# anerisheth19/CNN-MobileNet-V1-implementation-on-AWS-FPGA-using-OpenCL

Hardware: AMD Instinct MI355X
Metric: images/sec MobileNet-V1 1.0x224 fp32, batch 256; per-stage HBM GB/s vs roofline (higher is better)
Workload: dtype f32

## Files before the change

cnn-mobilenet-v1-implementation-on-aws-fpga-using-opencl_amd/csrc/mbn_abi.hip:

```cpp
#include "mbn_internal.h"

#include <initializer_list>
#include <new>

mbn_tunables g_mbn_tune;

namespace {

struct Span { const void *p; double bytes; const char *what; };

int span_check(mbn_context *ctx, const Span *sp, int n)
{
    std::lock_guard<std::mutex> lk(ctx->mu);
    if (ctx->allocs.empty()) return MBN_OK;
    for (int i = 0; i < n; i++) {
        if (!sp[i].p || sp[i].bytes <= 0) continue;
        const uintptr_t a = (uintptr_t)sp[i].p;
        auto it = ctx->allocs.upper_bound(a);
        if (it == ctx->allocs.begin()) continue;
        --it;
        if (a >= it->first + it->second) continue;
        const double room = (double)(it->first + it->second - a);
        if (sp[i].bytes > room) {
            snprintf(ctx->last_error, sizeof(ctx->last_error), "%s: call touches %.0f bytes, %.0f left in its %zu-byte mbn_alloc buffer",
// ... 1163 lines not shown
                              const void *fc_bias, int batch, int rows, int cols, int channels, int classes, int k, void *workspace,
                              size_t workspace_bytes, void *stream)
{
    if (!ctx || !topk_idx_i32 || !topk_prob_f32 || !logits || !in || !fc_w || !workspace || batch <= 0 || rows <= 0 || cols <= 0 || channels <= 0 ||
        classes <= 0 || k < 1 || k > 8)
        return MBN_EINVAL;
    if (batch > 4 || channels < 64 || channels > 1024 || (channels % 64) != 0 || classes > 1024) return MBN_EUNSUPPORTED;
    if (workspace_bytes < mbn_pool_fc_ws_bytes(channels, classes)) return MBN_EINVAL;
    hipStream_t s = stream ? (hipStream_t)stream : ctx->stream;
    MBN_SPANS(ctx, { in, 4.0 * batch * rows * cols * channels, "classifier_tail_fused input" }, { logits, 4.0 * batch * classes, "classifier_tail_fused logits" },
              { fc_w, 4.0 * classes * channels, "classifier_tail_fused filter" }, { workspace, (double)mbn_pool_fc_ws_bytes(channels, classes), "classifier_tail_fused workspace" },
              { probs, 4.0 * batch * classes, "classifier_tail_fused probs" }, { topk_idx_i32, 4.0 * batch * k, "classifier_tail_fused idx" },
              { topk_prob_f32, 4.0 * batch * k, "classifier_tail_fused prob" });
    Scope sc(ctx, s);
    return sc.finish(mbn_launch_f32_pool_fc(ctx, s, (float *)logits, (const float *)in, (const float *)fc_w, (const float *)fc_bias, workspace,
                                            batch, rows * cols, channels, classes, k, (float *)probs, (int32_t *)topk_idx_i32, (float *)topk_prob_f32));
}

static int stem_fused_impl(mbn_context *ctx, void *out, const void *image, const void *w1, const void *s1, const void *b1,
                           const void *wd, const void *s2, const void *b2, const void *wp, const void *s3, const void *b3,
                           int batch, int rows, int cols, int c1, int c3, void *stream, int in_u8, int bf16)
{
    if (!ctx || !out || !image) return MBN_EINVAL;
    hipStream_t s = stream ? (hipStream_t)stream : ctx->stream;
    if (mbn_stem_envelope_hw(batch, rows, cols, c1, c3) != MBN_OK) return MBN_EUNSUPPORTED;
    MBN_SPANS(ctx, { image, (in_u8 ? 1.0 : 4.0) * batch * rows * cols * 3, "stem image" },
              { out, (bf16 ? 2.0 : 4.0) * batch * (rows / 2) * (cols / 2) * c3, "stem output" });
    if (check_ptrs({ w1, s1, b1, wd, s2, b2, wp, s3, b3 }) != MBN_OK) return MBN_EUNSUPPORTED;
    if (((uintptr_t)out % 16) != 0 || ((uintptr_t)image % (in_u8 ? 2 : 8)) != 0) return MBN_EINVAL;
    Scope sc(ctx, s);
    return sc.finish(mbn_launch_f32_stem(ctx, s, (float *)out, (const float *)image, (const float *)w1, (const float *)s1,
                                         (const float *)b1, (const float *)wd, (const float *)s2, (const float *)b2,
                                         (const float *)wp, (const float *)s3, (const float *)b3, batch, rows, cols, c1, c3, in_u8, bf16));
}

int mbn_stem_fused_hw(mbn_context *ctx, void *out, const void *image, const void *w1, const void *s1, const void *b1,
                      const void *wd, const void *s2, const void *b2, const void *wp, const void *s3, const void *b3,
                      int batch, int rows, int cols, int c1, int c3, int flags, void *stream)
{
    if (flags & ~(MBN_STEM_IN_U8 | MBN_STEM_BF16)) return MBN_EINVAL;
    return stem_fused_impl(ctx, out, image, w1, s1, b1, wd, s2, b2, wp, s3, b3, batch, rows, cols, c1, c3, stream,
                           (flags & MBN_STEM_IN_U8) != 0, (flags & MBN_STEM_BF16) != 0);
}

int mbn_stem_fused(mbn_context *ctx, void *out, const void *image, const void *w1, const void *s1, const void *b1,
                   const void *wd, const void *s2, const void *b2, const void *wp, const void *s3, const void *b3,
                   int batch, int res, int c1, int c3, void *stream)
{
    return mbn_stem_fused_hw(ctx, out, image, w1, s1, b1, wd, s2, b2, wp, s3, b3, batch, res, res, c1, c3, 0, stream);
}

int mbn_stem_fused_u8(mbn_context *ctx, void *out, const void *image_u8, const void *w1, const void *s1, const void *b1,
                      const void *wd, const void *s2, const void *b2, const void *wp, const void *s3, const void *b3,
                      int batch, int res, int c1, int c3, void *stream)
{
    return mbn_stem_fused_hw(ctx, out, image_u8, w1, s1, b1, wd, s2, b2, wp, s3, b3, batch, res, res, c1, c3, MBN_STEM_IN_U8, stream);
}

int mbn_stem_fused_ex(mbn_context *ctx, void *out, const void *image, const void *w1, const void *s1, const void *b1,
                      const void *wd, const void *s2, const void *b2, const void *wp, const void *s3, const void *b3,
                      int batch, int res, int c1, int c3, int flags, void *stream)
{
    return mbn_stem_fused_hw(ctx, out, image, w1, s1, b1, wd, s2, b2, wp, s3, b3, batch, res, res, c1, c3, flags, stream);
}

int mbn_dwpw_fused(mbn_context *ctx, void *out, const void *in, const void *wd, const void *s2, const void *b2,
                   const void *wp, const void *s3, const void *b3, int batch, int in_rows, int in_cols, int out_rows,
                   int out_cols, int cin, int cout, int stride, int pad_top, int pad_left, void *stream)
{
    if (!ctx) return MBN_EINVAL;
    hipStream_t s = stream ? (hipStream_t)stream : ctx->stream;
    const mbn_block_shape sh = { batch, in_rows, in_cols, out_rows, out_cols, cin, cout, stride, pad_top, pad_left };
    const mbn_block_params p = { wd, s2, b2, wp, s3, b3 };
    int rc = check_ptrs({ in, wd, s2, b2, wp, s3, b3, out });
    if (rc == MBN_OK) rc = mbn_block_envelope(&sh, MBN_DT_F32);
    if (rc != MBN_OK) return rc;
    MBN_SPANS(ctx, { in, 4.0 * batch * in_rows * in_cols * cin, "dwpw input" },
              { out, 4.0 * batch * out_rows * out_cols * cout, "dwpw output" }, { wd, 36.0 * cin, "dwpw depthwise filter" },
              { wp, 4.0 * cin * cout, "dwpw pointwise filter" });
    Scope sc(ctx, s);
    if (g_mbn_tune.pw_emul != 0 && g_mbn_tune.dwpw_variant == 0 && mbn_launch_f32_dwpw2_x6(ctx, s, sh, out, in, p) == MBN_OK)
        return sc.finish(MBN_OK);
    const int dv = g_mbn_tune.dwpw_variant;
    if ((dv == 11 || dv >= 300 || (dv == 0 && MBN_DWPW3_DEFAULT(stride, cin))) && mbn_f32_dwpw3_eligible(ctx, sh))
        return sc.finish(mbn_launch_f32_dwpw3(ctx, s, sh, out, in, p));
    const long tiles256 = (((long)batch * out_rows * out_cols + 127) / 128) * (cout / 256);
    const bool small = tiles256 < ctx->num_cus;
    if (dv != 1 && (dv >= 2 || (cout % 256) != 0 || small || stride == 2))
        return sc.finish(mbn_launch_f32_dwpw2(ctx, s, sh, out, in, p));
    return sc.finish(mbn_launch_f32_dwpw(ctx, s, sh, out, in, p));
}

int mbn_blocks_resident_bf16(mbn_context *ctx, void *out, const void *in, const mbn_block_params *blocks, int nblocks, int batch,
                             int rows, int cols, int channels, void *stream)
{
    if (!ctx || !out || !in || !blocks || batch <= 0) return MBN_EINVAL;
    const mbn_block_shape sh = { batch, rows, cols, rows, cols, channels, channels, 1, 1, 1 };
    if (mbn_resident_envelope(&sh, nblocks) != MBN_OK) return MBN_EUNSUPPORTED;
    hipStream_t s = stream ? (hipStream_t)stream : ctx->stream;
    const double act = 2.0 * batch * rows * cols * channels;
    MBN_SPANS(ctx, { in, act, "resident blocks input" }, { out, act, "resident blocks output" });
    for (int i = 0; i < nblocks; i++) {
        if (!blocks[i].wd || !blocks[i].s2 || !blocks[i].b2 || !blocks[i].wp_bf16 || !blocks[i].s3 || !blocks[i].b3) return MBN_EINVAL;
        MBN_SPANS(ctx, { blocks[i].wd, 36.0 * channels, "resident blocks depthwise filter" }, { blocks[i].wp_bf16, 2.0 * channels * channels, "resident blocks pointwise filter" },
                  { blocks[i].s2, 4.0 * channels, "resident blocks scale" }, { blocks[i].b3, 4.0 * channels, "resident blocks shift" });
    }
    int rc = check_ptrs({ out, in });
    for (int i = 0; i < nblocks && rc == MBN_OK; i++) rc = check_ptrs(blocks[i]);
    if (rc != MBN_OK) return rc;
    Scope sc(ctx, s);
    return sc.finish(mbn_launch_bf16_res_blocks(ctx, s, out, in, blocks, nblocks, batch, rows, cols));
}

int mbn_tail_resident_bf16(mbn_context *ctx, void *out, const void *in, const mbn_block_params *blocks, int batch, int rows, int cols, int c0, int c1,
                           void *stream)
{
    if (!ctx || !out || !in || !blocks || batch <= 0) return MBN_EINVAL;
    const mbn_block_shape b0 = { batch, rows, cols, rows / 2, cols / 2, c0, c1, 2, 0, 0 };
    const mbn_block_shape b1 = { batch, rows / 2, cols / 2, rows / 2, cols / 2, c1, c1, 1, 1, 1 };
    if (mbn_tail_envelope(&b0, &b1) != MBN_OK) return MBN_EUNSUPPORTED;
    hipStream_t s = stream ? (hipStream_t)stream : ctx->stream;
    MBN_SPANS(ctx, { in, 2.0 * batch * rows * cols * c0, "resident tail input" }, { out, 2.0 * batch * c1, "resident tail output" });
    for (int i = 0; i < 2; i++) {
        if (!blocks[i].wd || !blocks[i].s2 || !blocks[i].b2 || !blocks[i].wp_bf16 || !blocks[i].s3 || !blocks[i].b3) return MBN_EINVAL;
        const int ci = i ? c1 : c0;
        MBN_SPANS(ctx, { blocks[i].wd, 36.0 * ci, "resident tail depthwise filter" }, { blocks[i].wp_bf16, 2.0 * ci * c1, "resident tail pointwise filter" },
                  { blocks[i].s2, 4.0 * ci, "resident tail scale" }, { blocks[i].b2, 4.0 * ci, "resident tail shift" },
                  { blocks[i].s3, 4.0 * c1, "resident tail scale" }, { blocks[i].b3, 4.0 * c1, "resident tail shift" });
    }
    int rc = ((uintptr_t)out % 2) ? MBN_EUNSUPPORTED : check_ptrs({ in });
    for (int i = 0; i < 2 && rc == MBN_OK; i++) rc = check_ptrs(blocks[i]);
    if (rc != MBN_OK) return rc;
    Scope sc(ctx, s);
    return sc.finish(mbn_launch_bf16_tail(ctx, s, out, in, blocks, batch, rows, cols));
}

int mbn_dwpw_fused_bf16(mbn_context *ctx, void *out, const void *in, const void *wd, const void *s2, const void *b2,
                        const void *wp_bf16, const void *s3, const void *b3, int batch, int in_rows, int in_cols, int out_rows,
                        int out_cols, int cin, int cout, int stride, int pad_top, int pad_left, void *stream)
{
    if (!ctx) return MBN_EINVAL;
    hipStream_t s = stream ? (hipStream_t)stream : ctx->stream;
    const mbn_block_shape sh = { batch, in_rows, in_cols, out_rows, out_cols, cin, cout, stride, pad_top, pad_left };
    const mbn_block_params p = { wd, s2, b2, wp_bf16, s3, b3 };
    int rc = check_ptrs({ in, wd, s2, b2, wp_bf16, s3, b3, out });
    if (rc == MBN_OK) rc = mbn_block_envelope(&sh, MBN_DT_BF16);
    if (rc != MBN_OK) return rc;
    MBN_SPANS(ctx, { in, 2.0 * batch * in_rows * in_cols * cin, "dwpw input" },
              { out, 2.0 * batch * out_rows * out_cols * cout, "dwpw output" }, { wd, 36.0 * cin, "dwpw depthwise filter" },
              { wp_bf16, 2.0 * cin * cout, "dwpw pointwise filter" });
    Scope sc(ctx, s);
#ifdef MBN_LAB
    if (g_mbn_tune.dwpw_variant == 1 && (cout % 128) == 0 && (cin % 64) == 0)
        return sc.finish(mbn_launch_bf16_dwpw(ctx, s, sh, out, in, p));
#endif
    return sc.finish(mbn_launch_bf16_dwpw2(ctx, s, sh, out, in, p));
}

int mbn_convert_f32_to_bf16(mbn_context *ctx, void *dst_bf16, const void *src_f32, size_t count, void *stream)
{
    if (!ctx || !dst_bf16 || !src_f32) return MBN_EINVAL;
    if (count == 0) return MBN_OK;
    hipStream_t s = stream ? (hipStream_t)stream : ctx->stream;
    MBN_SPANS(ctx, { src_f32, 4.0 * count, "convert source" }, { dst_bf16, 2.0 * count, "convert destination" });
    Scope sc(ctx, s);
    return sc.finish(mbn_launch_convert(ctx, s, dst_bf16, src_f32, count, 1));
}
// ... 46 lines not shown
```

cnn-mobilenet-v1-implementation-on-aws-fpga-using-opencl_amd/csrc/mbn_f32_dwpw3.hip:

```cpp
#include "mbn_internal.h"
#include "mbn_epilogue.h"
#include "mbn_block_window.h"

namespace {

constexpr int BN3 = 128;
constexpr int WT = 32;
constexpr unsigned PO_INVALID = MBN_OFF_BAD_ROW;

struct DwPw3Args {
    float *out;
    const float *in, *wd, *s2, *b2, *wp, *s3, *b3;
    long m;
    int h, w, ho, wo;
    int cout;
    int pad_top, pad_left;
    int nh;
    int tiles;
    unsigned in_bytes;
    int rsh;
    unsigned pb, bi;
    unsigned pb_m, pb_s, bi_m, bi_s;
    float inv_pb, inv_bi;
    int dbg;
};

__device__ __forceinline__ f4 bn_relu6_pk(f4 a, f4 s, f4 b)
{
    const f4 v = __builtin_elementwise_fma(a, s, b);
    return f4{ mbn_relu6(v.x), mbn_relu6(v.y), mbn_relu6(v.z), mbn_relu6(v.w) };
}

template <int S, int CIN, int KS, int ABL, int SCHED = 0, bool B64 = false>
__global__ __launch_bounds__(512) void dwpw3_f32(DwPw3Args a)
{
    constexpr int XC = S + 3;
    constexpr int NS = CIN / 16;
    constexpr int AH = KS / 16;
    constexpr int LPP = KS / 4;
    constexpr int LDB = B64 ? CIN + 2 : CIN + 4;
    constexpr int ABUF = WT * KS;
    static_assert(NS >= 4 && (CIN % 64) == 0 && (KS == 16 || KS == 32), "Cin in multiples of 64");
    __shared__ __attribute__((aligned(16))) float lds[BN3 * LDB + 8 * AH * ABUF + 11 * CIN + 2 * BN3 + 8 * 32];
    float *const wp_s = lds, *const a_s = wp_s + BN3 * LDB, *const wd_s = a_s + 8 * AH * ABUF, *const sb_s = wd_s + 9 * CIN;
    float *const sc3_s = sb_s + 2 * CIN, *const sh3_s = sc3_s + BN3;
    unsigned *const po_s = reinterpret_cast<unsigned *>(sh3_s + BN3);
    const int dbg = ABL < 0 ? a.dbg : ABL;

    const int tid = threadIdx.x, lane = tid & 63;
    const int wave_u = __builtin_amdgcn_readfirstlane(tid >> 6);
    const unsigned ptot = (unsigned)(a.m >> 1);

    const int xcd = (int)blockIdx.x & 7, j = (int)blockIdx.x >> 3, g8 = (int)gridDim.x >> 3;
    const int slice = j % a.nh, jm = j / a.nh, JM = g8 / a.nh;
    const int n0 = slice * BN3;
    const int r0 = (int)(((long)a.tiles * xcd) >> 3), r1 = (int)(((long)a.tiles * (xcd + 1)) >> 3);
    const int per_round = JM * 8;
    const int full = (r1 - r0) / per_round, rem = (r1 - r0) - full * per_round;
    const int slot = jm * 8 + wave_u, eslot = wave_u * JM + jm;
    const int ntile = full + (eslot < rem ? 1 : 0);
    auto tile_at = [&](int i) __attribute__((always_inline)) { return i < full ? r0 + i * per_round + slot : r0 + full * per_round + eslot; };

    {
        constexpr int NP = BN3 * (CIN / 4) / 512;
        f4 pc[NP];
#pragma unroll
        for (int i = 0; i < NP; i++) {
            const int p = tid + i * 512, r = p / (CIN / 4), u = p % (CIN / 4);
            const int ch = n0 + 4 * (r & 31) + (r >> 5);
            pc[i] = *reinterpret_cast<const f4 *>(a.wp + (size_t)ch * CIN + 4 * u);
        }
        f4 tp[3];
        const int ti = tid * 4;
#pragma unroll
        for (int i = 0; i < 3; i++) {
            const int idx = ti + i * 2048;
            tp[i] = idx < 9 * CIN ? *reinterpret_cast<const f4 *>(a.wd + idx) : f4{ 0.f, 0.f, 0.f, 0.f };
        }
        f4 sb[2] = { f4{ 0.f, 0.f, 0.f, 0.f }, f4{ 0.f, 0.f, 0.f, 0.f } };
        if (ti < CIN) {
            sb[0] = *reinterpret_cast<const f4 *>(a.s2 + ti);
            sb[1] = *reinterpret_cast<const f4 *>(a.b2 + ti);
        }
#pragma unroll
        for (int i = 0; i < NP; i++) {
            const int p = tid + i * 512, r = p / (CIN / 4), u = p % (CIN / 4);
            if constexpr (B64) {
                *reinterpret_cast<f2 *>(wp_s + r * LDB + 4 * u) = f2{ pc[i].x, pc[i].y };
                *reinterpret_cast<f2 *>(wp_s + r * LDB + 4 * u + 2) = f2{ pc[i].z, pc[i].w };
            } else *reinterpret_cast<f4 *>(wp_s + r * LDB + 4 * u) = pc[i];
        }
#pragma unroll
        for (int i = 0; i < 3; i++) {
            const int idx = ti + i * 2048;
            if (idx < 9 * CIN) *reinterpret_cast<f4 *>(wd_s + idx) = tp[i];
        }
        if (ti < CIN) {
            *reinterpret_cast<f4 *>(sb_s + ti) = sb[0];
            *reinterpret_cast<f4 *>(sb_s + CIN + ti) = sb[1];
        }
    }
    if (tid < BN3) { sc3_s[tid] = a.s3[n0 + tid]; sh3_s[tid] = a.b3[n0 + tid]; }
    __syncthreads();
    if (ntile == 0) return;

    const int qh = lane / LPP, cl = lane % LPP;
    const int li = lane & 31, lh = lane >> 5;
    const __amdgpu_buffer_rsrc_t irsrc = mbn_make_rsrc(a.in, a.in_bytes);
    const __amdgpu_buffer_rsrc_t orsrc = mbn_make_rsrc(a.out, (unsigned)(a.m * a.cout * 4));
    float *const a_w = a_s + wave_u * (AH * ABUF);
    unsigned *const po_w = po_s + wave_u * 32;
    auto aw_at = [&](const int hh) __attribute__((always_inline)) {
        const int row = 8 * hh * (AH - 1) + qh;
        return KS == 16 ? row * KS + ((cl ^ ((row >> 2) & 3)) << 2) : row * KS + ((cl ^ ((row >> 1) & 7)) << 2);
    };
    const int aw[2] = { aw_at(0), aw_at(1) };
    auto fra_at = [&](const int u) __attribute__((always_inline)) {
        return KS == 16 ? li * KS + (((u + lh) ^ ((li >> 2) & 3)) << 2) : li * KS + (((u + lh) ^ ((li >> 1) & 7)) << 2);
    };
    const int fra[4] = { fra_at(0), fra_at(2), fra_at(KS == 32 ? 4 : 0), fra_at(KS == 32 ? 6 : 2) };
    const float *const bl01 = wp_s + li * LDB + lh * 4;
    const float *const bl23 = bl01 + 64 * LDB;
    const float *const wk = wd_s + cl * 4;

    constexpr bool SEP = S == 2 && AH == 2;
    unsigned off[SEP ? 1 : AH][SEP ? 1 : 3][SEP ? 1 : XC];
    unsigned rowv_k[SEP ? AH : 1][3], colv_k[SEP ? AH : 1][XC];
    auto set_offsets = [&](unsigned p0, const int hh, int pslot) __attribute__((always_inline)) {
        const unsigned bg0 = a.pb_m ? __umulhi(p0, a.pb_m) >> a.pb_s : p0;
        const unsigned i0 = p0 - bg0 * a.pb;
        const unsigned im0 = a.bi_m ? __umulhi(bg0, a.bi_m) >> a.bi_s : bg0;
        const unsigned b0 = bg0 - im0 * a.bi;
        const unsigned qq = (unsigned)(8 * hh * (AH - 1) + qh);
        const unsigned i1 = i0 + qq;
        const unsigned dq = (unsigned)__builtin_fmaf((float)i1, a.inv_pb, 0.5f * a.inv_pb);
        const unsigned i = i1 - (unsigned)__mul24((int)dq, (int)a.pb);
        const unsigned b1 = b0 + dq;
        const unsigned dn = (unsigned)__builtin_fmaf((float)b1, a.inv_bi, 0.5f * a.inv_bi);
        const unsigned band = b1 - (unsigned)__mul24((int)dn, (int)a.bi);
        const unsigned n = im0 + dn;
        const unsigned y = (band << a.rsh) + (i & ((1u << a.rsh) - 1u)), x = (i >> a.rsh) << 1;
        const bool mok = p0 + qq < ptot;
        unsigned rowv[3], colv[XC];
        mbn_window_rowcol<S>(rowv, colv, a, (unsigned)CIN * 4u, (unsigned)(cl * 16), n, y, x, mok);
        if constexpr (SEP) {
#pragma unroll
            for (int dy = 0; dy < 3; dy++) rowv_k[hh][dy] = rowv[dy];
#pragma unroll
            for (int jj = 0; jj < XC; jj++) colv_k[hh][jj] = colv[jj];
        } else {
#pragma unroll
            for (int dy = 0; dy < 3; dy++)
#pragma unroll
                for (int jj = 0; jj < XC; jj++) off[hh][dy][jj] = rowv[dy] + colv[jj];
        }
        const unsigned opix = (unsigned)__mul24((int)(n * (unsigned)a.ho + y), a.wo) + x;
        const unsigned po = mok ? opix * ((unsigned)a.cout * 4u) : PO_INVALID;
        unsigned lid;
        asm volatile("v_mbcnt_lo_u32_b32 %0, -1, 0\n\tv_mbcnt_hi_u32_b32 %0, -1, %0" : "=v"(lid));
        if ((lid % LPP) == 0) po_w[pslot * 16 + 8 * hh * (AH - 1) + (int)(lid / LPP)] = po;
    };
    auto set_offsets_tile = [&](unsigned p0, int pslot) __attribute__((always_inline)) {
#pragma unroll
        for (int hh = 0; hh < AH; hh++) set_offsets(p0, hh, pslot);
    };

    f4 xr[3][XC];
    auto ldx_row = [&](const int u, const int dy) __attribute__((always_inline)) {
        const int hh = AH == 2 ? (u & 1) : 0, cb = AH == 2 ? (u >> 1) * 128 : u * 64;
#pragma unroll
        for (int jj = 0; jj < XC; jj++)
            xr[dy][jj] = __builtin_bit_cast(f4, __builtin_amdgcn_raw_buffer_load_b128(irsrc, (SEP ? rowv_k[hh][dy] + colv_k[hh][jj] : off[SEP ? 0 : hh][SEP ? 0 : dy][SEP ? 0 : jj]) + (unsigned)cb, 0, 0));
    };
    f4 wrow[3], wss[2];
    auto ldw_row = [&](const int u, const int dy) __attribute__((always_inline)) {
        if (dbg & 32) return;
        const int cf = AH == 2 ? (u >> 1) * 32 : u * 16;
#pragma unroll
        for (int dx = 0; dx < 3; dx++) wrow[dx] = *reinterpret_cast<const f4 *>(wk + cf + (dy * 3 + dx) * CIN);
    };
    auto ldw_ss = [&](const int u) __attribute__((always_inline)) {
        if (dbg & 32) return;
        const int cf = AH == 2 ? (u >> 1) * 32 : u * 16;
        wss[0] = *reinterpret_cast<const f4 *>(wk + 9 * CIN + cf);
        wss[1] = *reinterpret_cast<const f4 *>(wk + 10 * CIN + cf);
    };
    f4 dacc0 = f4{ 0.f, 0.f, 0.f, 0.f }, dacc1 = dacc0;
    auto dw_row = [&](const int u, const int dy) __attribute__((always_inline)) {
        if (dy == 0) {
            dacc0 = f4{ 0.f, 0.f, 0.f, 0.f };
            dacc1 = dacc0;
        }
        if (!(dbg & 2)) {
#pragma unroll
            for (int dx = 0; dx < 3; dx++) {
                dacc0 = __builtin_elementwise_fma(xr[dy][dx], wrow[dx], dacc0);
                dacc1 = __builtin_elementwise_fma(xr[dy][dx + S], wrow[dx], dacc1);
            }
        }
        if (dy < 2) ldw_row(u, dy + 1);
        else ldw_ss(u);
    };
    auto dw_fin = [&](const int u) __attribute__((always_inline)) {
        if (dbg & 64) return;
        const int hh = AH == 2 ? (u & 1) : 0, buf = AH == 2 ? ((u >> 1) & 1) * ABUF : 0;
        *reinterpret_cast<f4 *>(a_w + buf + aw[hh]) = bn_relu6_pk(dacc0, wss[0], wss[1]);
        *reinterpret_cast<f4 *>(a_w + buf + aw[hh] + 16 * KS) = bn_relu6_pk(dacc1, wss[0], wss[1]);
    };

    f16v acc[4];
    f4 fa[2], fb[B64 ? 1 : 2][B64 ? 1 : 4];
    f2 fbh[B64 ? 2 : 1][B64 ? 4 : 1];
    auto ldfrag_a = [&](const int u, const int g) __attribute__((always_inline)) {
        if (dbg & 128) return;
        const int buf = AH == 2 ? ((u >> 1) & 1) * ABUF : 0, idx = AH == 2 ? 2 * (u & 1) + g : g;
        fa[g] = *reinterpret_cast<const f4 *>(a_w + buf + fra[idx]);
    };
    auto ldfrag_bh = [&](const int u, const int G) __attribute__((always_inline)) {
        if (dbg & 128) return;
        const int o = u * 16 + (G >> 1) * 8 + (G & 1) * 2;
        fbh[B64 ? (G & 1) : 0][0] = *reinterpret_cast<const f2 *>(bl01 + o);
        fbh[B64 ? (G & 1) : 0][B64 ? 1 : 0] = *reinterpret_cast<const f2 *>(bl01 + 32 * LDB + o);
        fbh[B64 ? (G & 1) : 0][B64 ? 2 : 0] = *reinterpret_cast<const f2 *>(bl23 + o);
        fbh[B64 ? (G & 1) : 0][B64 ? 3 : 0] = *reinterpret_cast<const f2 *>(bl23 + 32 * LDB + o);
    };
    auto ldfrag_b = [&](const int u, const int g) __attribute__((always_inline)) {
        if (dbg & 128) return;
        if constexpr (B64) return;
        fb[g][0] = *reinterpret_cast<const f4 *>(bl01 + u * 16 + g * 8);
        fb[g][B64 ? 0 : 1] = *reinterpret_cast<const f4 *>(bl01 + 32 * LDB + u * 16 + g * 8);
        fb[g][B64 ? 0 : 2] = *reinterpret_cast<const f4 *>(bl23 + u * 16 + g * 8);
        fb[g][B64 ? 0 : 3] = *reinterpret_cast<const f4 *>(bl23 + 32 * LDB + u * 16 + g * 8);
    };
    auto mfma8 = [&](const int g, const int s0, const bool first) __attribute__((always_inline)) {
        if (dbg & 16) return;
        const f16v zero = { 0.f, 0.f, 0.f, 0.f, 0.f, 0.f, 0.f, 0.f, 0.f, 0.f, 0.f, 0.f, 0.f, 0.f, 0.f, 0.f };
#pragma unroll
        for (int s = s0; s < s0 + 2; s++)
#pragma unroll
            for (int t = 0; t < 4; t++)
                acc[t] = __builtin_amdgcn_mfma_f32_32x32x2f32(fa[g][s], B64 ? fbh[B64 ? ((2 * g + (s0 >> 1)) & 1) : 0][B64 ? t : 0][s & 1] : fb[B64 ? 0 : g][B64 ? 0 : t][s], (first && s == s0) ? zero : acc[t], 0, 0, 0);
    };
    auto epilogue = [&](int pslot) __attribute__((always_inline)) {
        if (dbg & 4) return;
        const f4 sc = *reinterpret_cast<const f4 *>(sc3_s + 4 * li), sh = *reinterpret_cast<const f4 *>(sh3_s + 4 * li);
        const u4 pa = *reinterpret_cast<const u4 *>(po_w + pslot * 16 + 4 * lh), pb4 = *reinterpret_cast<const u4 *>(po_w + pslot * 16 + 8 + 4 * lh);
        const unsigned lane_col = (unsigned)(n0 + 4 * li) * 4u;
        unsigned vo[2][4];
#pragma unroll
        for (int c = 0; c < 4; c++) {
            vo[0][c] = pa[c] + lane_col;
            vo[1][c] = pb4[c] + lane_col;
        }
        const unsigned rowb = (unsigned)a.cout * 4u;
#pragma unroll
        for (int r = 0; r < 16; r += 2) {
            f2 p[4];
#pragma unroll
            for (int t = 0; t < 4; t++) p[t] = __builtin_elementwise_fma(f2{ acc[t][r], acc[t][r + 1] }, f2{ sc[t], sc[t] }, f2{ sh[t], sh[t] });
            f4 o[2];
#pragma unroll
            for (int hh = 0; hh < 2; hh++)
                o[hh] = f4{ mbn_relu6(hh ? p[0].y : p[0].x), mbn_relu6(hh ? p[1].y : p[1].x), mbn_relu6(hh ? p[2].y : p[2].x), mbn_relu6(hh ? p[3].y : p[3].x) };
            __builtin_amdgcn_sched_barrier(0);
#pragma unroll
            for (int hh = 0; hh < 2; hh++) {
                const int rr = r + hh;
                __builtin_amdgcn_raw_buffer_store_b128(__builtin_bit_cast(u4, o[hh]), orsrc, vo[(rr >> 2) & 1][rr & 3], (rr >> 3) ? rowb : 0u, 0);
            }
            mbn_store_hazard_wait();
        }
    };

    int it = 0;
    unsigned p0M = (unsigned)tile_at(0) * 16u;
    set_offsets_tile(p0M, 0);
#pragma unroll
    for (int u = 0; u < AH; u++) {
#pragma unroll
        for (int dy = 0; dy < 3; dy++) ldx_row(u, dy);
        ldw_row(u, 0);
#pragma unroll
        for (int dy = 0; dy < 3; dy++) dw_row(u, dy);
        dw_fin(u);
    }
#pragma unroll
    for (int dy = 0; dy < 3; dy++) ldx_row(AH, dy);
    ldfrag_a(0, 0);
    ldfrag_b(0, 0);
    if constexpr (B64) ldfrag_bh(0, 0);
    ldw_row(AH, 0);
    bool pendE = false;

    for (;;) {
        const bool have_next = it + 1 < ntile;
        const unsigned p0N = have_next ? (unsigned)tile_at(it + 1) * 16u : p0M;
        if (SCHED != 3 && pendE) {
            epilogue((it - 1) & 1);
            pendE = false;
        }

#pragma unroll
        for (int u = 0; u < NS; u++) {
            const int ud = (u + AH) % NS, ul = (u + AH + 1) % NS;
            if (u == NS - AH - 1 && have_next && !(dbg & 256)) set_offsets_tile(p0N, (it + 1) & 1);
            if constexpr (SCHED == 3) {
                if (u == 0) {
                    __builtin_amdgcn_sched_barrier(0);
                    ldfrag_a(u, 1);
                    ldfrag_b(u, 1);
#pragma unroll
                    for (int dy = 0; dy < 3; dy++) {
                        dw_row(ud, dy);
                        if (!(dbg & 1)) ldx_row(ul, dy);
                    }
                    dw_fin(ud);
                    __builtin_amdgcn_sched_barrier(0);
                    if (pendE) {
                        epilogue((it - 1) & 1);
                        pendE = false;
                    }
                    __builtin_amdgcn_sched_barrier(0);
                    if constexpr (B64) ldfrag_bh(u, 1);
                    mfma8(0, 0, true);
                    __builtin_amdgcn_sched_barrier(0);
                    if constexpr (B64) ldfrag_bh(u, 2);
                    mfma8(0, 2, false);
                    __builtin_amdgcn_sched_barrier(0);
                    ldfrag_b((u + 1) % NS, 0);
                    if constexpr (B64) ldfrag_bh(u, 3);
                    __builtin_amdgcn_sched_barrier(0);
                    mfma8(1, 0, false);
                    __builtin_amdgcn_sched_barrier(0);
                    ldfrag_a((u + 1) % NS, 0);
                    if constexpr (B64) ldfrag_bh((u + 1) % NS, 0);
                    ldw_row(ul, 0);
                    __builtin_amdgcn_sched_barrier(0);
                    mfma8(1, 2, false);
                    __builtin_amdgcn_sched_barrier(0);
                    continue;
                }
            }
#define SB() do { if constexpr (SCHED == 0) __builtin_amdgcn_sched_barrier(0); } while (0)
            __builtin_amdgcn_sched_barrier(0);
            ldfrag_a(u, 1);
            ldfrag_b(u, 1);
            if constexpr (B64) ldfrag_bh(u, 1);
            dw_row(ud, 0);
            if (!(dbg & 1)) ldx_row(ul, 0);
            SB();
            mfma8(0, 0, u == 0);
            SB();
            if constexpr (B64) ldfrag_bh(u, 2);
            dw_row(ud, 1);
            if (!(dbg & 1)) ldx_row(ul, 1);
            SB();
            mfma8(0, 2, false);
            SB();
            ldfrag_b((u + 1) % NS, 0);
            if constexpr (B64) ldfrag_bh(u, 3);
            dw_row(ud, 2);
            if (!(dbg & 1)) ldx_row(ul, 2);
            SB();
            mfma8(1, 0, false);
            SB();
            dw_fin(ud);
            ldfrag_a((u + 1) % NS, 0);
            if constexpr (B64) ldfrag_bh((u + 1) % NS, 0);
            ldw_row(ul, 0);
            SB();
            mfma8(1, 2, false);
            if constexpr (SCHED == 2) {
#pragma unroll
                for (int i = 0; i < 32; i++) {
                    __builtin_amdgcn_sched_group_barrier(0x008, 1, 0);
                    __builtin_amdgcn_sched_group_barrier(0x002, 2, 0);
                    __builtin_amdgcn_sched_group_barrier(0x320, 1, 0);
                }
            }
            __builtin_amdgcn_sched_barrier(0);
#undef SB
        }
        pendE = true;
        if (!have_next) break;
        p0M = p0N;
        it++;
    }
    epilogue(it & 1);
}

template <int S, int CIN, int KS>
void launch3(const DwPw3Args &a, hipStream_t s, int grid)
{
#ifdef MBN_LAB
    if constexpr (S == 1 && ((CIN == 128 && KS == 32) || (CIN == 256 && KS == 16))) {
        switch (a.dbg) {
        case 1: hipLaunchKernelGGL((dwpw3_f32<S, CIN, KS, 1>), dim3((unsigned)grid), dim3(512), 0, s, a); return;
        case 2: hipLaunchKernelGGL((dwpw3_f32<S, CIN, KS, 2>), dim3((unsigned)grid), dim3(512), 0, s, a); return;
        case 4: hipLaunchKernelGGL((dwpw3_f32<S, CIN, KS, 4>), dim3((unsigned)grid), dim3(512), 0, s, a); return;
        case 7: hipLaunchKernelGGL((dwpw3_f32<S, CIN, KS, 7>), dim3((unsigned)grid), dim3(512), 0, s, a); return;
        case 16: hipLaunchKernelGGL((dwpw3_f32<S, CIN, KS, 16>), dim3((unsigned)grid), dim3(512), 0, s, a); return;
        case 23: hipLaunchKernelGGL((dwpw3_f32<S, CIN, KS, 23>), dim3((unsigned)grid), dim3(512), 0, s, a); return;
        case 39: hipLaunchKernelGGL((dwpw3_f32<S, CIN, KS, 39>), dim3((unsigned)grid), dim3(512), 0, s, a); return;
        case 103: hipLaunchKernelGGL((dwpw3_f32<S, CIN, KS, 103>), dim3((unsigned)grid), dim3(512), 0, s, a); return;
        case 231: hipLaunchKernelGGL((dwpw3_f32<S, CIN, KS, 231>), dim3((unsigned)grid), dim3(512), 0, s, a); return;
        case 487: hipLaunchKernelGGL((dwpw3_f32<S, CIN, KS, 487>), dim3((unsigned)grid), dim3(512), 0, s, a); return;
        case 503: hipLaunchKernelGGL((dwpw3_f32<S, CIN, KS, 503>), dim3((unsigned)grid), dim3(512), 0, s, a); return;
        default: break;
        }
    }
    if (a.dbg) { hipLaunchKernelGGL((dwpw3_f32<S, CIN, KS, -1>), dim3((unsigned)grid), dim3(512), 0, s, a); return; }
#endif
    hipLaunchKernelGGL((dwpw3_f32<S, CIN, KS, 0>), dim3((unsigned)grid), dim3(512), 0, s, a);
}

}

int mbn_f32_dwpw3_eligible(const mbn_context *ctx, const mbn_block_shape &s)
{
    if (s.cin != 64 && s.cin != 128 && s.cin != 256) return 0;
#ifndef MBN_LAB
    if (!MBN_DWPW3_DEFAULT(s.stride, s.cin)) return 0;
#endif
    if ((s.cout % BN3) != 0) return 0;
    if (mbn_block_fast_offsets(&s, MBN_DT_F32) != MBN_OK || s.out_cols >= 16384 || s.pad_top > 1) return 0;
    if ((double)s.batch * s.out_rows >= 2000000.0 || (double)s.batch * s.out_rows * s.out_cols >= 2147483000.0) return 0;
    if (4.0 * ((double)s.batch * s.out_rows * s.out_cols + WT) * s.cout > (double)PO_INVALID) return 0;
    const int nh = s.cout / BN3;
    if (ctx->num_cus / (8 * nh) < 1) return 0;
    return 1;
}

int mbn_launch_f32_dwpw3(mbn_context *ctx, hipStream_t stream, const mbn_block_shape &s, void *out, const void *in, const mbn_block_params &p)
{
    DwPw3Args a;
    a.out = (float *)out; a.in = (const float *)in; a.wd = (const float *)p.wd; a.s2 = (const float *)p.s2; a.b2 = (const float *)p.b2;
    a.wp = (const float *)p.wp_bf16; a.s3 = (const float *)p.s3; a.b3 = (const float *)p.b3;
    a.m = (long)s.batch * s.out_rows * s.out_cols;
    a.h = s.in_rows; a.w = s.in_cols; a.ho = s.out_rows; a.wo = s.out_cols;
    a.cout = s.cout; a.pad_top = s.pad_top; a.pad_left = s.pad_left;
    const int cin = s.cin, out_rows = s.out_rows, out_cols = s.out_cols;
    [[maybe_unused]] const int stride = s.stride;
    a.nh = s.cout / BN3;
    a.tiles = (int)((a.m + WT - 1) / WT);
    a.rsh = (out_rows % 4) == 0 ? 2 : (out_rows % 2) == 0 ? 1 : 0;
#ifdef MBN_LAB
    if (g_mbn_tune.exp1 >= 1 && g_mbn_tune.exp1 <= 3 && (out_rows % (1 << (g_mbn_tune.exp1 - 1))) == 0) a.rsh = g_mbn_tune.exp1 - 1;
#endif
    a.pb = (unsigned)((out_cols / 2) << a.rsh);
    a.bi = (unsigned)(out_rows >> a.rsh);
    mbn_udiv_magic(a.pb, &a.pb_m, &a.pb_s);
    mbn_udiv_magic(a.bi, &a.bi_m, &a.bi_s);
    a.inv_pb = 1.0f / (float)a.pb;
    a.inv_bi = 1.0f / (float)a.bi;
    a.in_bytes = (unsigned)(4.0 * s.batch * s.in_rows * s.in_cols * s.cin);
    const int variant = g_mbn_tune.dwpw_variant;
    a.dbg = variant >= 300 ? variant - 300 : 0;
    int per_xcd = ctx->num_cus / 8;
    per_xcd -= per_xcd % a.nh;
    const long tiles_xcd = (a.tiles + 7) / 8;
    if ((long)per_xcd > tiles_xcd * a.nh) per_xcd = (int)(tiles_xcd * a.nh);
    const int grid = per_xcd * 8;
    [[maybe_unused]] bool ks32 = cin <= 128;
#ifdef MBN_LAB
    if (g_mbn_tune.exp0 == 16) ks32 = false;
    if (!ks32 && cin <= 128) {
        if (stride == 1) { if (cin == 64) launch3<1, 64, 16>(a, stream, grid); else launch3<1, 128, 16>(a, stream, grid); }
        else { if (cin == 64) launch3<2, 64, 16>(a, stream, grid); else launch3<2, 128, 16>(a, stream, grid); }
        return MBN_OK;
    }
#endif
#ifdef MBN_LAB
    if (stride == 1 && g_mbn_tune.exp2 == 5 && !a.dbg && cin >= 128) {
        if (cin == 128) hipLaunchKernelGGL((dwpw3_f32<1, 128, 32, 0, 3, true>), dim3((unsigned)grid), dim3(512), 0, stream, a);
        else hipLaunchKernelGGL((dwpw3_f32<1, 256, 16, 0, 3, true>), dim3((unsigned)grid), dim3(512), 0, stream, a);
        return MBN_OK;
    }
    if (stride == 1 && g_mbn_tune.exp2 == 4 && !a.dbg && cin >= 128) {
        if (cin == 128) hipLaunchKernelGGL((dwpw3_f32<1, 128, 32, 0, 0, true>), dim3((unsigned)grid), dim3(512), 0, stream, a);
        else hipLaunchKernelGGL((dwpw3_f32<1, 256, 16, 0, 0, true>), dim3((unsigned)grid), dim3(512), 0, stream, a);
        return MBN_OK;
    }
    if (stride == 1 && g_mbn_tune.exp2 >= 1 && g_mbn_tune.exp2 <= 3 && !a.dbg && cin >= 128) {
        const int sc = g_mbn_tune.exp2;
        if (cin == 128) {
            if (sc == 1) hipLaunchKernelGGL((dwpw3_f32<1, 128, 32, 0, 1>), dim3((unsigned)grid), dim3(512), 0, stream, a);
            else if (sc == 2) hipLaunchKernelGGL((dwpw3_f32<1, 128, 32, 0, 2>), dim3((unsigned)grid), dim3(512), 0, stream, a);
            else hipLaunchKernelGGL((dwpw3_f32<1, 128, 32, 0, 3>), dim3((unsigned)grid), dim3(512), 0, stream, a);
        } else {
            if (sc == 1) hipLaunchKernelGGL((dwpw3_f32<1, 256, 16, 0, 1>), dim3((unsigned)grid), dim3(512), 0, stream, a);
            else if (sc == 2) hipLaunchKernelGGL((dwpw3_f32<1, 256, 16, 0, 2>), dim3((unsigned)grid), dim3(512), 0, stream, a);
            else hipLaunchKernelGGL((dwpw3_f32<1, 256, 16, 0, 3>), dim3((unsigned)grid), dim3(512), 0, stream, a);
        }
        return MBN_OK;
    }
#endif
#ifdef MBN_LAB
    if (stride == 1) {
        if (cin == 64) launch3<1, 64, 32>(a, stream, grid);
        else if (cin == 128) launch3<1, 128, 32>(a, stream, grid);
        else launch3<1, 256, 16>(a, stream, grid);
    } else {
        if (cin == 64) launch3<2, 64, 32>(a, stream, grid);
        else if (cin == 128) launch3<2, 128, 32>(a, stream, grid);
        else launch3<2, 256, 16>(a, stream, grid);
    }
#else
    if (cin == 128) launch3<1, 128, 32>(a, stream, grid);
    else launch3<1, 256, 16>(a, stream, grid);
#endif
    return MBN_OK;
}
```

Measured before the change: 91200.

## Add 2x2 output-patch depthwise form to fused f32 dw+pw kernel for Cin≤128

Adds a PATCH template variant of the fused depthwise+pointwise f32 kernel. Each lane computes a 2x2 output patch (two rows, two columns), so the overlapping 3x3 input window rows are loaded once and shared between vertically adjacent outputs. The patch loop is interleaved with the MFMA pointwise schedule. Tile and row-band bookkeeping (ptot, bi rounding, rsh) is changed to count pixel pairs, and eligibility excludes shapes where the patch would read past the padded width. The aim is fewer redundant global loads for the depthwise stage, at the cost of more registers and a more complex schedule.

Result: no change. 91600, median of 6 (+0.4%).

```diff
diff --git a/cnn-mobilenet-v1-implementation-on-aws-fpga-using-opencl_amd/csrc/mbn_abi.hip b/cnn-mobilenet-v1-implementation-on-aws-fpga-using-opencl_amd/csrc/mbn_abi.hip
--- a/cnn-mobilenet-v1-implementation-on-aws-fpga-using-opencl_amd/csrc/mbn_abi.hip
+++ b/cnn-mobilenet-v1-implementation-on-aws-fpga-using-opencl_amd/csrc/mbn_abi.hip
@@ -1269,7 +1269,7 @@
     if (g_mbn_tune.pw_emul != 0 && g_mbn_tune.dwpw_variant == 0 && mbn_launch_f32_dwpw2_x6(ctx, s, sh, out, in, p) == MBN_OK)
         return sc.finish(MBN_OK);
     const int dv = g_mbn_tune.dwpw_variant;
-    if ((dv == 11 || dv >= 300 || (dv == 0 && MBN_DWPW3_DEFAULT(stride, cin))) && mbn_f32_dwpw3_eligible(ctx, sh))
+    if ((dv == 11 || dv == 13 || dv >= 300 ||(dv == 0 && MBN_DWPW3_DEFAULT(stride, cin))) && mbn_f32_dwpw3_eligible(ctx, sh))
         return sc.finish(mbn_launch_f32_dwpw3(ctx, s, sh, out, in, p));
     const long tiles256 = (((long)batch * out_rows * out_cols + 127) / 128) * (cout / 256);
     const bool small = tiles256 < ctx->num_cus;
diff --git a/cnn-mobilenet-v1-implementation-on-aws-fpga-using-opencl_amd/csrc/mbn_f32_dwpw3.hip b/cnn-mobilenet-v1-implementation-on-aws-fpga-using-opencl_amd/csrc/mbn_f32_dwpw3.hip
--- a/cnn-mobilenet-v1-implementation-on-aws-fpga-using-opencl_amd/csrc/mbn_f32_dwpw3.hip
+++ b/cnn-mobilenet-v1-implementation-on-aws-fpga-using-opencl_amd/csrc/mbn_f32_dwpw3.hip
@@ -17,6 +17,7 @@
     int pad_top, pad_left;
     int nh;
     int tiles;
+    unsigned ptot;
     unsigned in_bytes;
     int rsh;
     unsigned pb, bi;
@@ -31,7 +32,7 @@
     return f4{ mbn_relu6(v.x), mbn_relu6(v.y), mbn_relu6(v.z), mbn_relu6(v.w) };
 }
 
-template <int S, int CIN, int KS, int ABL, int SCHED = 0, bool B64 = false>
+template <int S, int CIN, int KS, int ABL, int SCHED = 0, bool B64 = false, bool PATCH = false>
 __global__ __launch_bounds__(512) void dwpw3_f32(DwPw3Args a)
 {
     constexpr int XC = S + 3;
@@ -41,6 +42,8 @@
     constexpr int LDB = B64 ? CIN + 2 : CIN + 4;
     constexpr int ABUF = WT * KS;
     static_assert(NS >= 4 && (CIN % 64) == 0 && (KS == 16 || KS == 32), "Cin in multiples of 64");
+    static_assert(!PATCH || (S == 1 && KS == 32 && SCHED == 0), "the 2x2 patch form: stride 1, 32-channel chunks, the pinned schedule");
+    constexpr int NC = NS / 2;
     __shared__ __attribute__((aligned(16))) float lds[BN3 * LDB + 8 * AH * ABUF + 11 * CIN + 2 * BN3 + 8 * 32];
     float *const wp_s = lds, *const a_s = wp_s + BN3 * LDB, *const wd_s = a_s + 8 * AH * ABUF, *const sb_s = wd_s + 9 * CIN;
     float *const sc3_s = sb_s + 2 * CIN, *const sh3_s = sc3_s + BN3;
@@ -49,7 +52,7 @@
 
     const int tid = threadIdx.x, lane = tid & 63;
     const int wave_u = __builtin_amdgcn_readfirstlane(tid >> 6);
-    const unsigned ptot = (unsigned)(a.m >> 1);
+    const unsigned ptot = a.ptot;
 
     const int xcd = (int)blockIdx.x & 7, j = (int)blockIdx.x >> 3, g8 = (int)gridDim.x >> 3;
     const int slice = j % a.nh, jm = j / a.nh, JM = g8 / a.nh;
@@ -160,9 +163,45 @@
         asm volatile("v_mbcnt_lo_u32_b32 %0, -1, 0\n\tv_mbcnt_hi_u32_b32 %0, -1, %0" : "=v"(lid));
         if ((lid % LPP) == 0) po_w[pslot * 16 + 8 * hh * (AH - 1) + (int)(lid / LPP)] = po;
     };
+    unsigned poff[PATCH ? 4 : 1][3];
+    auto set_offsets_patch = [&](unsigned p0, int pslot) __attribute__((always_inline)) {
+        const unsigned bg0 = a.pb_m ? __umulhi(p0, a.pb_m) >> a.pb_s : p0;
+        const unsigned i0 = p0 - bg0 * a.pb;
+        const unsigned im0 = a.bi_m ? __umulhi(bg0, a.bi_m) >> a.bi_s : bg0;
+        const unsigned b0 = bg0 - im0 * a.bi;
+        const unsigned qq = (unsigned)(2 * qh);
+        const unsigned i1 = i0 + qq;
+        const unsigned dq = (unsigned)__builtin_fmaf((float)i1, a.inv_pb, 0.5f * a.inv_pb);
+        const unsigned i = i1 - (unsigned)__mul24((int)dq, (int)a.pb);
+        const unsigned b1 = b0 + dq;
+        const unsigned dn = (unsigned)__builtin_fmaf((float)b1, a.inv_bi, 0.5f * a.inv_bi);
+        const unsigned band = b1 - (unsigned)__mul24((int)dn, (int)a.bi);
+        const unsigned n = im0 + dn;
+        const unsigned y = (band << a.rsh) + (i & ((1u << a.rsh) - 1u)), x = (i >> a.rsh) << 1;
+        const bool oku = p0 + qq < ptot, okl = oku && y + 1u < (unsigned)a.ho;
+        unsigned rowu[3], rowl[3], colv[XC], colw[XC];
+        mbn_window_rowcol<S>(rowu, colv, a, (unsigned)CIN * 4u, (unsigned)(cl * 16), n, y, x, oku);
+        mbn_window_rowcol<S>(rowl, colw, a, (unsigned)CIN * 4u, (unsigned)(cl * 16), n, y + 1u, x, oku);
+#pragma unroll
+        for (int r = 0; r < (PATCH ? 4 : 1); r++) {
+            const unsigned rv = r < 3 ? rowu[r] : rowl[2];
+            poff[r][0] = rv + colv[0];
+            poff[r][1] = rv + colv[1];
+            poff[r][2] = rv + colv[XC - 1];
+        }
+        const unsigned opix = (unsigned)__mul24((int)(n * (unsigned)a.ho + y), a.wo) + x;
+        const unsigned rowb = (unsigned)a.cout * 4u;
+        const u2 po = { oku ? opix * rowb : PO_INVALID, okl ? (opix + (unsigned)a.wo) * rowb : PO_INVALID };
+        unsigned lid;
+        asm volatile("v_mbcnt_lo_u32_b32 %0, -1, 0\n\tv_mbcnt_hi_u32_b32 %0, -1, %0" : "=v"(lid));
+        if ((lid % LPP) == 0) *reinterpret_cast<u2 *>(po_w + pslot * 16 + 2 * (int)(lid / LPP)) = po;
+    };
     auto set_offsets_tile = [&](unsigned p0, int pslot) __attribute__((always_inline)) {
-#pragma unroll
-        for (int hh = 0; hh < AH; hh++) set_offsets(p0, hh, pslot);
+        if constexpr (PATCH) set_offsets_patch(p0, pslot);
+        else {
+#pragma unroll
+            for (int hh = 0; hh < AH; hh++) set_offsets(p0, hh, pslot);
+        }
     };
 
     f4 xr[3][XC];
@@ -206,6 +245,48 @@
         const int hh = AH == 2 ? (u & 1) : 0, buf = AH == 2 ? ((u >> 1) & 1) * ABUF : 0;
         *reinterpret_cast<f4 *>(a_w + buf + aw[hh]) = bn_relu6_pk(dacc0, wss[0], wss[1]);
         *reinterpret_cast<f4 *>(a_w + buf + aw[hh] + 16 * KS) = bn_relu6_pk(dacc1, wss[0], wss[1]);
+    };
+
+    f4 xp[PATCH ? 4 : 1][XC];
+    f4 du0 = f4{ 0.f, 0.f, 0.f, 0.f }, du1 = du0, dl0 = du0, dl1 = du0;
+    auto ldx_prow = [&](const int c, const int r) __attribute__((always_inline)) {
+        constexpr unsigned PIX = (unsigned)CIN * 4u;
+        const unsigned cb = (unsigned)c * 128u;
+        xp[r][0] = __builtin_bit_cast(f4, __builtin_amdgcn_raw_buffer_load_b128(irsrc, poff[r][0] + cb, 0, 0));
+        xp[r][1] = __builtin_bit_cast(f4, __builtin_amdgcn_raw_buffer_load_b128(irsrc, poff[r][1] + cb, 0, 0));
+        xp[r][2] = __builtin_bit_cast(f4, __builtin_amdgcn_raw_buffer_load_b128(irsrc, poff[r][1] + (PIX + cb), 0, 0));
+        xp[r][XC - 1] = __builtin_bit_cast(f4, __builtin_amdgcn_raw_buffer_load_b128(irsrc, poff[r][2] + cb, 0, 0));
+    };
+    auto ldw_prow = [&](const int c, const int dy) __attribute__((always_inline)) {
+        if (dbg & 32) return;
+#pragma unroll
+        for (int dx = 0; dx < 3; dx++) wrow[dx] = *reinterpret_cast<const f4 *>(wk + c * 32 + (dy * 3 + dx) * CIN);
+    };
+    auto ldw_pss = [&](const int c) __attribute__((always_inline)) {
+        if (dbg & 32) return;
+        wss[0] = *reinterpret_cast<const f4 *>(wk + 9 * CIN + c * 32);
+        wss[1] = *reinterpret_cast<const f4 *>(wk + 10 * CIN + c * 32);
+    };
+    auto dw_prow = [&](f4 &s0, f4 &s1, const int r, const bool start) __attribute__((always_inline)) {
+        if (start) {
+            s0 = f4{ 0.f, 0.f, 0.f, 0.f };
+            s1 = s0;
+        }
+        if (dbg & 2) return;
+#pragma unroll
+        for (int dx = 0; dx < 3; dx++) {
+            s0 = __builtin_elementwise_fma(xp[r][dx], wrow[dx], s0);
+            s1 = __builtin_elementwise_fma(xp[r][dx + 1], wrow[dx], s1);
+        }
+    };
+    const int awp = 2 * qh * KS + ((cl ^ (qh & 7)) << 2);
+    auto dw_pfin = [&](const int c) __attribute__((always_inline)) {
+        if (dbg & 64) return;
+        float *const t = a_w + (c & 1) * ABUF + awp;
+        *reinterpret_cast<f4 *>(t) = bn_relu6_pk(du0, wss[0], wss[1]);
+        *reinterpret_cast<f4 *>(t + 16 * KS) = bn_relu6_pk(du1, wss[0], wss[1]);
+        *reinterpret_cast<f4 *>(t + KS) = bn_relu6_pk(dl0, wss[0], wss[1]);
+        *reinterpret_cast<f4 *>(t + 17 * KS) = bn_relu6_pk(dl1, wss[0], wss[1]);
     };
 
     f16v acc[4];
@@ -275,21 +356,40 @@
     int it = 0;
     unsigned p0M = (unsigned)tile_at(0) * 16u;
     set_offsets_tile(p0M, 0);
-#pragma unroll
-    for (int u = 0; u < AH; u++) {
-#pragma unroll
-        for (int dy = 0; dy < 3; dy++) ldx_row(u, dy);
-        ldw_row(u, 0);
-#pragma unroll
-        for (int dy = 0; dy < 3; dy++) dw_row(u, dy);
-        dw_fin(u);
-    }
-#pragma unroll
-    for (int dy = 0; dy < 3; dy++) ldx_row(AH, dy);
+    if constexpr (PATCH) {
+#pragma unroll
+        for (int r = 0; r < 4; r++) ldx_prow(0, r);
+        ldw_prow(0, 0);
+        dw_prow(du0, du1, 0, true);
+        dw_prow(dl0, dl1, 1, true);
+        ldw_prow(0, 1);
+        dw_prow(du0, du1, 1, false);
+        dw_prow(dl0, dl1, 2, false);
+        ldw_prow(0, 2);
+        dw_prow(du0, du1, 2, false);
+        dw_prow(dl0, dl1, 3, false);
+        ldw_pss(0);
+        dw_pfin(0);
+#pragma unroll
+        for (int r = 0; r < 4; r++) ldx_prow(1, r);
+    } else {
+#pragma unroll
+        for (int u = 0; u < AH; u++) {
+#pragma unroll
+            for (int dy = 0; dy < 3; dy++) ldx_row(u, dy);
+            ldw_row(u, 0);
+#pragma unroll
+            for (int dy = 0; dy < 3; dy++) dw_row(u, dy);
+            dw_fin(u);
+        }
+#pragma unroll
+        for (int dy = 0; dy < 3; dy++) ldx_row(AH, dy);
+    }
     ldfrag_a(0, 0);
     ldfrag_b(0, 0);
     if constexpr (B64) ldfrag_bh(0, 0);
-    ldw_row(AH, 0);
+    if constexpr (PATCH) ldw_prow(1, 0);
+    else ldw_row(AH, 0);
     bool pendE = false;
 
     for (;;) {
@@ -303,7 +403,56 @@
 #pragma unroll
         for (int u = 0; u < NS; u++) {
             const int ud = (u + AH) % NS, ul = (u + AH + 1) % NS;
-            if (u == NS - AH - 1 && have_next && !(dbg & 256)) set_offsets_tile(p0N, (it + 1) & 1);
+            if (u == (PATCH ? NS - 4 : NS - AH - 1) && have_next && !(dbg & 256)) set_offsets_tile(p0N, (it + 1) & 1);
+            if constexpr (PATCH) {
+                const int cd = ((u >> 1) + 1) % NC, cn = ((u >> 1) + 2) % NC;
+                const bool ld = !(dbg & 1);
+                __builtin_amdgcn_sched_barrier(0);
+                ldfrag_a(u, 1);
+                ldfrag_b(u, 1);
+                if constexpr (B64) ldfrag_bh(u, 1);
+                if ((u & 1) == 0) {
+                    dw_prow(du0, du1, 0, true);
+                    if (ld) ldx_prow(cn, 0);
+                } else {
+                    dw_prow(du0, du1, 2, false);
+                    if (ld) ldx_prow(cn, 2);
+                }
+                __builtin_amdgcn_sched_barrier(0);
+                mfma8(0, 0, u == 0);
+                __builtin_amdgcn_sched_barrier(0);
+                if constexpr (B64) ldfrag_bh(u, 2);
+                if ((u & 1) == 0) {
+                    dw_prow(dl0, dl1, 1, true);
+                    ldw_prow(cd, 1);
+                } else {
+                    dw_prow(dl0, dl1, 3, false);
+                    if (ld) ldx_prow(cn, 3);
+                    ldw_pss(cd);
+                }
+                __builtin_amdgcn_sched_barrier(0);
+                mfma8(0, 2, false);
+                __builtin_amdgcn_sched_barrier(0);
+                ldfrag_b((u + 1) % NS, 0);
+                if constexpr (B64) ldfrag_bh(u, 3);
+                if ((u & 1) == 0) {
+                    dw_prow(du0, du1, 1, false);
+                    if (ld) ldx_prow(cn, 1);
+                } else dw_pfin(cd);
+                __builtin_amdgcn_sched_barrier(0);
+                mfma8(1, 0, false);
+                __builtin_amdgcn_sched_barrier(0);
+                if ((u & 1) == 0) {
+                    dw_prow(dl0, dl1, 2, false);
+                    ldw_prow(cd, 2);
+                } else ldw_prow(cn, 0);
+                ldfrag_a((u + 1) % NS, 0);
+                if constexpr (B64) ldfrag_bh((u + 1) % NS, 0);
+                __builtin_amdgcn_sched_barrier(0);
+                mfma8(1, 2, false);
+                __builtin_amdgcn_sched_barrier(0);
+                continue;
+            }
             if constexpr (SCHED == 3) {
                 if (u == 0) {
                     __builtin_amdgcn_sched_barrier(0);
@@ -389,29 +538,29 @@
     epilogue(it & 1);
 }
 
-template <int S, int CIN, int KS>
+template <int S, int CIN, int KS, bool PATCH = false>
 void launch3(const DwPw3Args &a, hipStream_t s, int grid)
 {
 #ifdef MBN_LAB
     if constexpr (S == 1 && ((CIN == 128 && KS == 32) || (CIN == 256 && KS == 16))) {
         switch (a.dbg) {
-        case 1: hipLaunchKernelGGL((dwpw3_f32<S, CIN, KS, 1>), dim3((unsigned)grid), dim3(512), 0, s, a); return;
-        case 2: hipLaunchKernelGGL((dwpw3_f32<S, CIN, KS, 2>), dim3((unsigned)grid), dim3(512), 0, s, a); return;
-        case 4: hipLaunchKernelGGL((dwpw3_f32<S, CIN, KS, 4>), dim3((unsigned)grid), dim3(512), 0, s, a); return;
-        case 7: hipLaunchKernelGGL((dwpw3_f32<S, CIN, KS, 7>), dim3((unsigned)grid), dim3(512), 0, s, a); return;
-        case 16: hipLaunchKernelGGL((dwpw3_f32<S, CIN, KS, 16>), dim3((unsigned)grid), dim3(512), 0, s, a); return;
-        case 23: hipLaunchKernelGGL((dwpw3_f32<S, CIN, KS, 23>), dim3((unsigned)grid), dim3(512), 0, s, a); return;
-        case 39: hipLaunchKernelGGL((dwpw3_f32<S, CIN, KS, 39>), dim3((unsigned)grid), dim3(512), 0, s, a); return;
-        case 103: hipLaunchKernelGGL((dwpw3_f32<S, CIN, KS, 103>), dim3((unsigned)grid), dim3(512), 0, s, a); return;
-        case 231: hipLaunchKernelGGL((dwpw3_f32<S, CIN, KS, 231>), dim3((unsigned)grid), dim3(512), 0, s, a); return;
-        case 487: hipLaunchKernelGGL((dwpw3_f32<S, CIN, KS, 487>), dim3((unsigned)grid), dim3(512), 0, s, a); return;
-        case 503: hipLaunchKernelGGL((dwpw3_f32<S, CIN, KS, 503>), dim3((unsigned)grid), dim3(512), 0, s, a); return;
+        case 1: hipLaunchKernelGGL((dwpw3_f32<S, CIN, KS, 1, 0, PATCH, PATCH>), dim3((unsigned)grid), dim3(512), 0, s, a); return;
+        case 2: hipLaunchKernelGGL((dwpw3_f32<S, CIN, KS, 2, 0, PATCH, PATCH>), dim3((unsigned)grid), dim3(512), 0, s, a); return;
+        case 4: hipLaunchKernelGGL((dwpw3_f32<S, CIN, KS, 4, 0, PATCH, PATCH>), dim3((unsigned)grid), dim3(512), 0, s, a); return;
+        case 7: hipLaunchKernelGGL((dwpw3_f32<S, CIN, KS, 7, 0, PATCH, PATCH>), dim3((unsigned)grid), dim3(512), 0, s, a); return;
+        case 16: hipLaunchKernelGGL((dwpw3_f32<S, CIN, KS, 16, 0, PATCH, PATCH>), dim3((unsigned)grid), dim3(512), 0, s, a); return;
+        case 23: hipLaunchKernelGGL((dwpw3_f32<S, CIN, KS, 23, 0, PATCH, PATCH>), dim3((unsigned)grid), dim3(512), 0, s, a); return;
+        case 39: hipLaunchKernelGGL((dwpw3_f32<S, CIN, KS, 39, 0, PATCH, PATCH>), dim3((unsigned)grid), dim3(512), 0, s, a); return;
+        case 103: hipLaunchKernelGGL((dwpw3_f32<S, CIN, KS, 103, 0, PATCH, PATCH>), dim3((unsigned)grid), dim3(512), 0, s, a); return;
+        case 231: hipLaunchKernelGGL((dwpw3_f32<S, CIN, KS, 231, 0, PATCH, PATCH>), dim3((unsigned)grid), dim3(512), 0, s, a); return;
+        case 487: hipLaunchKernelGGL((dwpw3_f32<S, CIN, KS, 487, 0, PATCH, PATCH>), dim3((unsigned)grid), dim3(512), 0, s, a); return;
+        case 503: hipLaunchKernelGGL((dwpw3_f32<S, CIN, KS, 503, 0, PATCH, PATCH>), dim3((unsigned)grid), dim3(512), 0, s, a); return;
         default: break;
         }
     }
-    if (a.dbg) { hipLaunchKernelGGL((dwpw3_f32<S, CIN, KS, -1>), dim3((unsigned)grid), dim3(512), 0, s, a); return; }
+    if (a.dbg) { hipLaunchKernelGGL((dwpw3_f32<S, CIN, KS, -1, 0, PATCH, PATCH>), dim3((unsigned)grid), dim3(512), 0, s, a); return; }
 #endif
-    hipLaunchKernelGGL((dwpw3_f32<S, CIN, KS, 0>), dim3((unsigned)grid), dim3(512), 0, s, a);
+    hipLaunchKernelGGL((dwpw3_f32<S, CIN, KS, 0, 0, PATCH, PATCH>), dim3((unsigned)grid), dim3(512), 0, s, a);
 }
 
 }
@@ -425,6 +574,7 @@
     if ((s.cout % BN3) != 0) return 0;
     if (mbn_block_fast_offsets(&s, MBN_DT_F32) != MBN_OK || s.out_cols >= 16384 || s.pad_top > 1) return 0;
     if ((double)s.batch * s.out_rows >= 2000000.0 || (double)s.batch * s.out_rows * s.out_cols >= 2147483000.0) return 0;
+    if (s.stride == 1 && s.cin <= 128 && s.out_cols > s.in_cols + s.pad_left - 1) return 0;
     if (4.0 * ((double)s.batch * s.out_rows * s.out_cols + WT) * s.cout > (double)PO_INVALID) return 0;
     const int nh = s.cout / BN3;
     if (ctx->num_cus / (8 * nh) < 1) return 0;
@@ -442,20 +592,25 @@
     const int cin = s.cin, out_rows = s.out_rows, out_cols = s.out_cols;
     [[maybe_unused]] const int stride = s.stride;
     a.nh = s.cout / BN3;
-    a.tiles = (int)((a.m + WT - 1) / WT);
-    a.rsh = (out_rows % 4) == 0 ? 2 : (out_rows % 2) == 0 ? 1 : 0;
+    const int variant = g_mbn_tune.dwpw_variant;
+    a.dbg = variant >= 300 ? variant - 300 : 0;
+    bool patch = stride == 1 && cin <= 128;
 #ifdef MBN_LAB
-    if (g_mbn_tune.exp1 >= 1 && g_mbn_tune.exp1 <= 3 && (out_rows % (1 << (g_mbn_tune.exp1 - 1))) == 0) a.rsh = g_mbn_tune.exp1 - 1;
+    if (variant == 13 || g_mbn_tune.exp0 == 16 || (g_mbn_tune.exp2 >= 1 && g_mbn_tune.exp2 <= 5 && !a.dbg && cin >= 128)) patch = false;
+#endif
+    a.rsh = (out_rows % 4) == 0 ? 2 : ((out_rows % 2) == 0 || patch) ? 1 : 0;
+#ifdef MBN_LAB
+    if (g_mbn_tune.exp1 >= (patch ? 2 : 1) && g_mbn_tune.exp1 <= 3 && (out_rows % (1 << (g_mbn_tune.exp1 - 1))) == 0) a.rsh = g_mbn_tune.exp1 - 1;
 #endif
     a.pb = (unsigned)((out_cols / 2) << a.rsh);
-    a.bi = (unsigned)(out_rows >> a.rsh);
+    a.bi = (unsigned)((out_rows + (1 << a.rsh) - 1) >> a.rsh);
+    a.ptot = (unsigned)((long)s.batch * a.bi * a.pb);
+    a.tiles = (int)(((long)a.ptot + WT / 2 - 1) / (WT / 2));
     mbn_udiv_magic(a.pb, &a.pb_m, &a.pb_s);
     mbn_udiv_magic(a.bi, &a.bi_m, &a.bi_s);
     a.inv_pb = 1.0f / (float)a.pb;
     a.inv_bi = 1.0f / (float)a.bi;
     a.in_bytes = (unsigned)(4.0 * s.batch * s.in_rows * s.in_cols * s.cin);
-    const int variant = g_mbn_tune.dwpw_variant;
-    a.dbg = variant >= 300 ? variant - 300 : 0;
     int per_xcd = ctx->num_cus / 8;
     per_xcd -= per_xcd % a.nh;
     const long tiles_xcd = (a.tiles + 7) / 8;
@@ -497,8 +652,8 @@
 #endif
 #ifdef MBN_LAB
     if (stride == 1) {
-        if (cin == 64) launch3<1, 64, 32>(a, stream, grid);
-        else if (cin == 128) launch3<1, 128, 32>(a, stream, grid);
+        if (cin == 64) { if (patch) launch3<1, 64, 32, true>(a, stream, grid); else launch3<1, 64, 32>(a, stream, grid); }
+        else if (cin == 128) { if (patch) launch3<1, 128, 32, true>(a, stream, grid); else launch3<1, 128, 32>(a, stream, grid); }
         else launch3<1, 256, 16>(a, stream, grid);
     } else {
         if (cin == 64) launch3<2, 64, 32>(a, stream, grid);
@@ -506,7 +661,7 @@
         else launch3<2, 256, 16>(a, stream, grid);
     }
 #else
-    if (cin == 128) launch3<1, 128, 32>(a, stream, grid);
+    if (cin == 128) launch3<1, 128, 32, true>(a, stream, grid);
     else launch3<1, 256, 16>(a, stream, grid);
 #endif
     return MBN_OK;
```
